# broadinstitute/permutect

Hardware: AMD Instinct MI355X
Metric: read-sets/sec (train fwd+bwd) (higher is better)
Workload: dtype f32 (fp32 accumulate; fwd: 2 x f16 pieces per operand = 23 bits; bwd: 2 x bf16 pieces = 16 bits)

## Files before the change

### permutect_amd/csrc/pmt_cnn3.hip

```cpp
#define PMT_OWN_WAVE_SHAPE
#define PMT_WAVES 8
#define PMT_RT 1
#include "pmt_device.hpp"

#ifndef C3_FWD_V
#define C3_FWD_V 4
#define C3_FWD_NW 8
#endif
#define C3_BWD_V 8
#define C3_BWD_NW 4
#define C3_MAXK 7
#define C3_NACC(K1, K2, L2) ((K1) * 2 + (K2) * 4 + (L2) * 2)
#define C3_NBIAS 80

struct C3Cfg {
    int S, K1, L1, P1, K2, L2, C1, C2, F, O;
    int st1, st2;
    int n1t, n2t, nPt;
    int act1, act2;
    int w1, b1, w2, b2, wl, bl;
    int per_wave;
    int stash_per;
};

DEV void c3_wave_sync() {
    asm volatile("s_waitcnt lgkmcnt(0)" ::: "memory");
    __builtin_amdgcn_wave_barrier();
}
DEV int c3_row(int m) { return 4 * (m & 3) + (m >> 2); }
DEV float c3_act(int kind, float x) { return kind == PMT_CNN_LEAKY_RELU ? fmaxf(x, 0.01f * x) : selu1(x); }
DEV float c3_act_grad(int kind, float y) { return kind == PMT_CNN_LEAKY_RELU ? (y > 0.f ? 1.f : 0.01f) : selu_grad_from_out(y); }
DEV f4 c3_act4(int kind, f4 v) { return f4{c3_act(kind, v[0]), c3_act(kind, v[1]), c3_act(kind, v[2]), c3_act(kind, v[3])}; }
DEV f4 c3_act_grad4(int kind, f4 y) { return f4{c3_act_grad(kind, y[0]), c3_act_grad(kind, y[1]), c3_act_grad(kind, y[2]), c3_act_grad(kind, y[3])}; }
DEV f4 c3_mfma4(f4 a, f4 b, f4 c) {
#pragma unroll
    for (int j = 0; j < 4; ++j) c = mfma16(a[j], b[j], c);
    return c;
}
DEV f4 c3_zero() { return f4{0.f, 0.f, 0.f, 0.f}; }
template <int CTRL>
DEV f4 c3_dpp4(f4 v) { return f4{dpp_mov<CTRL>(v[0]), dpp_mov<CTRL>(v[1]), dpp_mov<CTRL>(v[2]), dpp_mov<CTRL>(v[3])}; }

struct C3Weights {
    const float *w1f, *w2f, *wlf;
    const float *w2tf, *wltf;
    const float *b1p, *b2p, *blp;
};
DEV int c3_weight_floats(const C3Cfg& c, bool backward) {
    const int fwd = c.K1 * 2 * 256 + c.K2 * 4 * 256 + c.L2 * 2 * 256 + 80;
    const int bwd = c.K2 * 4 * 256 + c.L2 * 2 * 256;
    return backward ? bwd : fwd;
}
DEV C3Weights c3_build_weights(const C3Cfg& c, const float* __restrict__ theta, float* __restrict__ lds, bool backward) {
    C3Weights W{};
    const int tid = threadIdx.x, nthr = blockDim.x;
    float* cur = lds;
    if (!backward) {
        float* w1f = cur; cur += c.K1 * 2 * 256;
        for (int i = tid; i < c.K1 * 2 * 256; i += nthr) {
            const int j = i & 3, lane = (i >> 2) & 63, mt = (i >> 8) & 1, tap = i >> 9;
            const int co = 16 * mt + c3_row(lane & 15), ci = 4 * j + (lane >> 4);
            w1f[i] = (co < c.C1 && ci < 10) ? theta[c.w1 + (co * 10 + ci) * c.K1 + tap] : 0.f;
        }
        float* w2f = cur; cur += c.K2 * 4 * 256;
        for (int i = tid; i < c.K2 * 4 * 256; i += nthr) {
            const int j = i & 3, lane = (i >> 2) & 63, kt = (i >> 8) & 1, mt = (i >> 9) & 1, tap = i >> 10;
            const int co = 16 * mt + c3_row(lane & 15), ci = 16 * kt + 4 * j + (lane >> 4);
            w2f[i] = (co < c.C2 && ci < c.C1) ? theta[c.w2 + (co * c.C1 + ci) * c.K2 + tap] : 0.f;
        }
        float* wlf = cur; cur += c.L2 * 2 * 256;
        for (int i = tid; i < c.L2 * 2 * 256; i += nthr) {
            const int j = i & 3, lane = (i >> 2) & 63, t = (i >> 8) & 1, p = i >> 9;
            const int o = c3_row(lane & 15), ch = 16 * t + 4 * j + (lane >> 4);
            wlf[i] = (o < c.O && ch < c.C2) ? theta[c.wl + o * c.F + ch * c.L2 + p] : 0.f;
        }
        float* bp = cur; cur += 80;
        for (int i = tid; i < 80; i += nthr) {
            const int e = i & 15, f = 16 * ((i >> 4) & 1) + c3_row(e);
            float v = 0.f;
            if (i < 32) v = f < c.C1 ? theta[c.b1 + f] : 0.f;
            else if (i < 64) v = f < c.C2 ? theta[c.b2 + f] : 0.f;
            else v = c3_row(e) < c.O ? theta[c.bl + c3_row(e)] : 0.f;
            bp[i] = v;
        }
        W.w1f = w1f; W.w2f = w2f; W.wlf = wlf; W.b1p = bp; W.b2p = bp + 32; W.blp = bp + 64;
    } else {
        float* w2tf = cur; cur += c.K2 * 4 * 256;
        for (int i = tid; i < c.K2 * 4 * 256; i += nthr) {
            const int j = i & 3, lane = (i >> 2) & 63, kt = (i >> 8) & 1, mt = (i >> 9) & 1, tap = i >> 10;
            const int ci = 16 * mt + c3_row(lane & 15), co = 16 * kt + 4 * j + (lane >> 4);
            w2tf[i] = (co < c.C2 && ci < c.C1) ? theta[c.w2 + (co * c.C1 + ci) * c.K2 + tap] : 0.f;
        }
        float* wltf = cur; cur += c.L2 * 2 * 256;
        for (int i = tid; i < c.L2 * 2 * 256; i += nthr) {
            const int j = i & 3, lane = (i >> 2) & 63, t = (i >> 8) & 1, p = i >> 9;
            const int ch = 16 * t + c3_row(lane & 15), o = 4 * j + (lane >> 4);
            wltf[i] = (o < c.O && ch < c.C2) ? theta[c.wl + o * c.F + ch * c.L2 + p] : 0.f;
        }
        W.w2tf = w2tf; W.wltf = wltf;
    }
    __syncthreads();
    return W;
}

#define C3_COPY_F4 20
#define C3_HAP_LOADS 8
struct C3Wave {
    float* rec;
    int rec_floats, a2_off, arg_off;
    float* x;
    float* dout;
    unsigned char* hap;
    int P1, st2;
    DEV float* a1(int v, int q) const { return rec + v * rec_floats + q * 32; }
    DEV float* a2(int v, int p) const { return rec + v * rec_floats + a2_off + p * 32; }
    DEV unsigned* argb(int v, int q) const { return reinterpret_cast<unsigned*>(rec + v * rec_floats + arg_off) + q; }
};
template <int V>
DEV C3Wave c3_wave_region(const C3Cfg& c, float* base) {
    C3Wave w;
    w.rec = base;
    w.rec_floats = c.stash_per;
    w.a2_off = c.P1 * 32;
    w.arg_off = c.P1 * 32 + c.st2 * 32;
    w.P1 = c.P1; w.st2 = c.st2;
    w.x = base + V * c.stash_per;
    w.dout = w.x + V * c.st2 * 32;
    w.hap = reinterpret_cast<unsigned char*>(w.dout + V * 16);
    return w;
}
template <int V>
DEV void c3_load_haplotypes(const C3Cfg& c, const C3Wave& w, const long long* __restrict__ hap, long long hap_stride, long long v0, int nv) {
    const int lane = threadIdx.x & 63, n2s = 2 * c.S;
    long long b[C3_HAP_LOADS];
#pragma unroll
    for (int k = 0; k < C3_HAP_LOADS; ++k) {
        const int i = lane + 64 * k, v = i / n2s, e = i - v * n2s;
        b[k] = 255;
        if (i < V * n2s && v < nv) b[k] = hap[(size_t)(v0 + v) * hap_stride + e];
    }
#pragma unroll
    for (int k = 0; k < C3_HAP_LOADS; ++k) {
        const int i = lane + 64 * k;
        if (i < V * n2s) w.hap[i] = (b[k] >= 0 && b[k] < 5) ? (unsigned char)b[k] : (unsigned char)255;
    }
}
DEV void c3_store_records(const C3Wave& w, float* __restrict__ dst, int nv) {
    const int lane = threadIdx.x & 63, have = nv * w.rec_floats / 4;
#pragma unroll
    for (int k = 0; k < C3_COPY_F4; ++k) {
        const int i = lane + 64 * k;
        if (i < have) reinterpret_cast<f4*>(dst)[i] = reinterpret_cast<const f4*>(w.rec)[i];
    }
}
DEV f4 c3_one_hot(int S, const C3Wave& w, int v, int pos, int g) {
    const int base = w.hap[v * 2 * S + (g & 1) * S + pos];
    const int b0 = g >> 1;
    return f4{base == b0 ? 1.f : 0.f, base == b0 + 2 ? 1.f : 0.f, (g < 2 && base == b0 + 4) ? 1.f : 0.f, 0.f};
}

#ifndef C3_TRACE
#define C3_TRACE 0
#endif
#define C3_EV()                                                                                                      \
    do {                                                                                                             \
        if (C3_TRACE && tracing) { const unsigned long long t_ = __builtin_readcyclecounter(); if (lane == 0 && tr_n < 120) tr[tr_n] = t_; ++tr_n; } \
    } while (0)
template <int V, int NW, int K1, int K2, int L2, int S1>
__global__ __launch_bounds__(64 * NW, 1) void pmt_cnn3_forward_kernel(
    C3Cfg c, const float* __restrict__ theta, const long long* __restrict__ hap, long long hap_stride, int n, float* __restrict__ out,
    long long out_stride, float* __restrict__ stash) {
    extern __shared__ __attribute__((aligned(16))) float lds[];
    const unsigned long long t_begin = C3_TRACE ? __builtin_readcyclecounter() : 0ull;
    const C3Weights W = c3_build_weights(c, theta, lds, false);
    const unsigned long long t_weights = C3_TRACE ? __builtin_readcyclecounter() : 0ull;
    const int lane = threadIdx.x & 63, g = lane >> 4, r = lane & 15, wave = uniform((int)(threadIdx.x >> 6));
    bool tracing = false;
    unsigned long long* tr = reinterpret_cast<unsigned long long*>(stash);
    int tr_n = 2;
    const C3Wave w = c3_wave_region<V>(c, lds + ((c3_weight_floats(c, false) + 3) & ~3) + wave * c.per_wave);
    const int nbatches = (n + V - 1) / V;
    constexpr int P1 = L2 + K2 - 1, ST2 = L2 <= 4 ? 4 : 8, N2T = (V * ST2 + 15) / 16;
    const int S = S1 ? S1 : c.S, st1 = S1 ? ((S1 - K1 + 2) & ~1) : c.st1, n1t = S1 ? (V * st1 + 15) / 16 : c.n1t;
    const float inv_st1 = 1.0f / (float)st1;
    const f4 b1v[2] = {*reinterpret_cast<const f4*>(W.b1p + 4 * g), *reinterpret_cast<const f4*>(W.b1p + 16 + 4 * g)};
    const f4 b2v[2] = {*reinterpret_cast<const f4*>(W.b2p + 4 * g), *reinterpret_cast<const f4*>(W.b2p + 16 + 4 * g)};
    const f4 blv = *reinterpret_cast<const f4*>(W.blp + 4 * g);
    for (int batch = blockIdx.x * NW + wave; batch < nbatches; batch += gridDim.x * NW) {
        const long long v0 = (long long)batch * V;
        const int nv = (int)min((long long)V, (long long)n - v0);
        C3_EV();
        c3_load_haplotypes<V>(c, w, hap, hap_stride, v0, nv);
        c3_wave_sync();
        C3_EV();
#pragma unroll
        for (int T = 0; T < n1t; ++T) {
            const int col = 16 * T + r;
            int v = S1 ? col / st1 : (int)((float)col * inv_st1 + 1e-3f);
            int p = col - v * st1;
            const bool in_range = v < V;
            v = min(v, V - 1);
            f4 acc[2] = {b1v[0], b1v[1]};
#pragma unroll
            for (int tap = 0; tap < K1; ++tap) {
                const f4 b = c3_one_hot(S, w, v, min(p + tap, S - 1), g);
#pragma unroll
                for (int mt = 0; mt < 2; ++mt) {
                    const f4 a = *reinterpret_cast<const f4*>(W.w1f + ((tap * 2 + mt) * 64 + lane) * 4);
#pragma unroll
                    for (int j = 0; j < 3; ++j) acc[mt] = mfma16(a[j], b[j], acc[mt]);
                }
            }
            const int q = p >> 1;
            const bool store = in_range && !(p & 1) && q < P1;
            unsigned bits = 0;
#pragma unroll
            for (int mt = 0; mt < 2; ++mt) {
                const f4 nxt = c3_dpp4<0x101>(acc[mt]);
                f4 m;
#pragma unroll
                for (int j = 0; j < 4; ++j) {
                    const bool second = nxt[j] > acc[mt][j];
                    m[j] = second ? nxt[j] : acc[mt][j];
                    bits |= second ? 1u << (4 * mt + j) : 0u;
                }
                if (store) *reinterpret_cast<f4*>(w.a1(v, q) + 16 * mt + 4 * g) = c3_act4(c.act1, m);
            }
            if (store) reinterpret_cast<unsigned char*>(w.argb(v, q))[g] = (unsigned char)bits;
        }
        c3_wave_sync();
        C3_EV();
#pragma unroll
        for (int T = 0; T < N2T; ++T) {
            const int col = 16 * T + r;
            int v = col / ST2;
            const int p = col - v * ST2;
            const bool valid = v < V && p < L2;
            v = min(v, V - 1);
            f4 acc[2] = {b2v[0], b2v[1]};
#pragma unroll
            for (int tap = 0; tap < K2; ++tap) {
                const float* src = w.a1(v, min(p + tap, P1 - 1)) + 4 * g;
#pragma unroll
                for (int kt = 0; kt < 2; ++kt) {
                    const f4 b = *reinterpret_cast<const f4*>(src + 16 * kt);
#pragma unroll
                    for (int mt = 0; mt < 2; ++mt)
                        acc[mt] = c3_mfma4(*reinterpret_cast<const f4*>(W.w2f + (((tap * 2 + mt) * 2 + kt) * 64 + lane) * 4), b, acc[mt]);
                }
            }
            if (v < V && p < ST2 && col < V * ST2) {
#pragma unroll
                for (int mt = 0; mt < 2; ++mt) *reinterpret_cast<f4*>(w.a2(v, p) + 16 * mt + 4 * g) = valid ? c3_act4(c.act2, acc[mt]) : c3_zero();
            }
        }
        c3_wave_sync();
        C3_EV();
        {
            const int v = min(r, V - 1);
            f4 acc = blv;
#pragma unroll
            for (int p = 0; p < L2; ++p)
#pragma unroll
                for (int t = 0; t < 2; ++t)
                    acc = c3_mfma4(*reinterpret_cast<const f4*>(W.wlf + ((p * 2 + t) * 64 + lane) * 4),
                                   *reinterpret_cast<const f4*>(w.a2(v, p) + 16 * t + 4 * g), acc);
            if (r < nv) {
#pragma unroll
                for (int j = 0; j < 4; ++j)
                    if (4 * j + g < c.O) out[(size_t)(v0 + r) * out_stride + 4 * j + g] = acc[j];
            }
        }
        C3_EV();
        if (stash) {
            c3_wave_sync();
            c3_store_records(w, stash + (size_t)v0 * c.stash_per, nv);
        }
        c3_wave_sync();
        if (C3_TRACE && stash != nullptr && blockIdx.x == 0 && wave == 0) {
            asm volatile("s_waitcnt vmcnt(0)" ::: "memory");
            if (!tracing && lane == 0) { tr[0] = t_begin; tr[1] = t_weights; }
            tracing = true;
            C3_EV();
            if (lane == 0) tr[127] = (unsigned long long)tr_n;
        }
    }
}

#define C3B_OH_PAD 16
DEV int c3_chan_of_elem(int e) { return 16 * (e >> 4) + 4 * (e & 3) + ((e & 15) >> 2); }
typedef unsigned c3_u4 __attribute__((ext_vector_type(4)));
typedef unsigned c3_u2 __attribute__((ext_vector_type(2)));
typedef h8 c3p8;
#define C3_NP 2
#define C3_ONE ((unsigned short)0x3C00)
DEV f4 c3p_mfma(c3p8 a, c3p8 b, f4 c) { return mfma_f16(a, b, c); }
DEV void c3p_split(float a, float b, unsigned (&pc)[3]) {
    float k = 4096.f;
    asm volatile("" : "+v"(k));
    split_pair_f16(a, b, pc[0], pc[1], k);
    pc[2] = 0u;
}
DEV void c3p_mma(const c3p8 (&a)[C3_NP], const c3p8 (&b)[C3_NP], f4& acc, f4& lo) {
    lo = c3p_mfma(a[1], b[0], lo);
    lo = c3p_mfma(a[0], b[1], lo);
    acc = c3p_mfma(a[0], b[0], acc);
}
DEV f4 c3p_join(f4 acc, f4 lo) { return lo * (1.0f / 4096.f) + acc; }
#define C3_COL_BYTES (64 * C3_NP)
template <typename F>
DEV void c3b_build_frag(c3p8* __restrict__ dst, int ln, F value) {
    unsigned pc[4][3];
#pragma unroll
    for (int q = 0; q < 4; ++q) c3p_split(value(2 * q), value(2 * q + 1), pc[q]);
#pragma unroll
    for (int k = 0; k < C3_NP; ++k) dst[64 * k + ln] = __builtin_bit_cast(c3p8, c3_u4{pc[0][k], pc[1][k], pc[2][k], pc[3][k]});
}
DEV void c3b_store_pieces(unsigned char* dst, f4 v) {
    unsigned p0[3], p1[3];
    c3p_split(v[0], v[1], p0);
    c3p_split(v[2], v[3], p1);
#pragma unroll
    for (int k = 0; k < C3_NP; ++k) *reinterpret_cast<c3_u2*>(dst + 64 * k) = c3_u2{p0[k], p1[k]};
}
__host__ __device__ inline size_t c3b_wave_bytes(int V, int S, int P1, int ST2) {
    return (size_t)((V * (S * 10 + C3B_OH_PAD) * 2 + 15) & ~15) + (size_t)V * P1 * C3_COL_BYTES + (size_t)V * ST2 * C3_COL_BYTES;
}

template <int V, int NW, int K1, int K2, int L2, int S1, int A1, int A2, bool TRAIN>
__global__ __launch_bounds__(64 * NW, 1) void pmt_cnn3_forward_bf_kernel(
    C3Cfg c, const float* __restrict__ theta, const long long* __restrict__ hap, long long hap_stride, int n, float* __restrict__ out,
    long long out_stride, float* __restrict__ stash) {
    static_assert(K1 * 10 <= 32, "conv1's taps x channels are one k block");
    extern __shared__ __attribute__((aligned(16))) float lds[];
    constexpr int P1 = L2 + K2 - 1, ST2 = L2 <= 4 ? 4 : 8, N2T = (V * ST2 + 15) / 16;
    const int tid = threadIdx.x, lane = tid & 63, g = lane >> 4, r = lane & 15, wave = uniform((int)(tid >> 6));
    const int S = S1 ? S1 : c.S, st1 = S1 ? ((S1 - K1 + 2) & ~1) : c.st1, n1t = S1 ? (V * st1 + 15) / 16 : c.n1t;
    const float inv_st1 = 1.0f / (float)st1;
    const int OHS = S * 10 + C3B_OH_PAD;
    unsigned char* base = reinterpret_cast<unsigned char*>(lds);
    fp16_saturate_on();
    c3p8* wlb = reinterpret_cast<c3p8*>(base);
    float* bp = reinterpret_cast<float*>(base + L2 * C3_NP * 1024);
    unsigned char* dyn = base + L2 * C3_NP * 1024 + 320;
    c3p8* w1s = reinterpret_cast<c3p8*>(dyn);
    c3p8* w2s = w1s + 2 * 64 * C3_NP;
    for (int e = tid; e < 2 * 64; e += 64 * NW) {
        const int ln = e & 63, mt = e >> 6, co = 16 * mt + c3_row(ln & 15), kg = ln >> 4;
        c3b_build_frag(w1s + mt * 64 * C3_NP, ln, [&](int i) {
            const int k = 8 * kg + i, tap = k / 10, ci = k - 10 * tap;
            return (k < 10 * K1 && co < c.C1) ? theta[c.w1 + (co * 10 + ci) * K1 + tap] : 0.f;
        });
    }
    for (int e = tid; e < K2 * 2 * 64; e += 64 * NW) {
        const int ln = e & 63, tm = e >> 6, tap = tm >> 1, mt = tm & 1, co = 16 * mt + c3_row(ln & 15), kg = ln >> 4;
        c3b_build_frag(w2s + tm * 64 * C3_NP, ln, [&](int i) {
            const int ci = c3_chan_of_elem(8 * kg + i);
            return (co < c.C2 && ci < c.C1) ? theta[c.w2 + (co * c.C1 + ci) * K2 + tap] : 0.f;
        });
    }
    for (int e = tid; e < L2 * 64; e += 64 * NW) {
        const int ln = e & 63, p = e >> 6, o = c3_row(ln & 15), kg = ln >> 4;
        c3b_build_frag(wlb + p * 64 * C3_NP, ln, [&](int i) {
            const int ch = c3_chan_of_elem(8 * kg + i);
            return (o < c.O && ch < c.C2) ? theta[c.wl + o * c.F + ch * L2 + p] : 0.f;
        });
    }
    for (int i = tid; i < 80; i += 64 * NW) {
        const int e = i & 15, f = 16 * ((i >> 4) & 1) + c3_row(e);
        float v = 0.f;
        if (i < 32) v = f < c.C1 ? theta[c.b1 + f] : 0.f;
        else if (i < 64) v = f < c.C2 ? theta[c.b2 + f] : 0.f;
        else v = c3_row(e) < c.O ? theta[c.bl + c3_row(e)] : 0.f;
        bp[i] = v;
    }
    __syncthreads();
    c3p8 w1r[2][C3_NP], w2r[K2][2][C3_NP];
#pragma unroll
    for (int mt = 0; mt < 2; ++mt)
#pragma unroll
        for (int pc = 0; pc < C3_NP; ++pc) w1r[mt][pc] = w1s[(mt * C3_NP + pc) * 64 + lane];
#pragma unroll
    for (int tap = 0; tap < K2; ++tap)
#pragma unroll
        for (int mt = 0; mt < 2; ++mt)
#pragma unroll
            for (int pc = 0; pc < C3_NP; ++pc) w2r[tap][mt][pc] = w2s[((tap * 2 + mt) * C3_NP + pc) * 64 + lane];
    const f4 b1v[2] = {*reinterpret_cast<const f4*>(bp + 4 * g), *reinterpret_cast<const f4*>(bp + 16 + 4 * g)};
    const f4 b2v[2] = {*reinterpret_cast<const f4*>(bp + 32 + 4 * g), *reinterpret_cast<const f4*>(bp + 48 + 4 * g)};
    const f4 blv = *reinterpret_cast<const f4*>(bp + 64 + 4 * g);
    __syncthreads();
    unsigned char* oh = dyn + (size_t)wave * c3b_wave_bytes(V, S, P1, ST2);
    unsigned char* a1b = oh + ((V * OHS * 2 + 15) & ~15);
    unsigned char* a2b = a1b + V * P1 * C3_COL_BYTES;
    for (int i = lane; i < (V * OHS) / 2; i += 64) reinterpret_cast<unsigned*>(oh)[i] = 0u;
    c3_wave_sync();
    const int nbatches = (n + V - 1) / V, n2s = 2 * S;
    const int rec_a2 = P1 * 32, rec_arg = P1 * 32 + ST2 * 32;
    long long bnext[C3_HAP_LOADS];
    auto request = [&](int batch) {
        const long long v0 = (long long)batch * V;
#pragma unroll
        for (int k = 0; k < C3_HAP_LOADS; ++k) {
            const int i = lane + 64 * k, v = i / n2s, e = i - v * n2s;
            bnext[k] = 255;
            if (batch < nbatches && i < V * n2s && v0 + v < n) bnext[k] = hap[(size_t)(v0 + v) * hap_stride + e];
        }
    };
    request(blockIdx.x * NW + wave);
    for (int batch = blockIdx.x * NW + wave; batch < nbatches; batch += gridDim.x * NW) {
        const long long v0 = (long long)batch * V;
        const int nv = (int)min((long long)V, (long long)n - v0);
        {
            long long b[C3_HAP_LOADS];
#pragma unroll
            for (int k = 0; k < C3_HAP_LOADS; ++k) b[k] = bnext[k];
            request(batch + gridDim.x * NW);
#pragma unroll
            for (int k = 0; k < C3_HAP_LOADS; ++k) {
                const int i = lane + 64 * k, v = i / n2s, e = i - v * n2s, hs = e >= S ? 1 : 0, pos = e - hs * S;
                if (i < V * n2s) {
                    unsigned short* dst = reinterpret_cast<unsigned short*>(oh) + v * OHS + pos * 10 + hs;
#pragma unroll
                    for (int bs = 0; bs < 5; ++bs) dst[2 * bs] = b[k] == bs ? C3_ONE : (unsigned short)0;
                }
            }
        }
        c3_wave_sync();
        float* rec0 = TRAIN ? stash + (size_t)v0 * c.stash_per : nullptr;
#pragma unroll
        for (int T = 0; T < n1t; ++T) {
            const int col = 16 * T + r;
            int v = S1 ? col / st1 : (int)((float)col * inv_st1 + 1e-3f);
            const int p = col - v * st1;
            const bool in_range = v < V;
            v = min(v, V - 1);
            const unsigned* src = reinterpret_cast<const unsigned*>(oh + 2 * (v * OHS + p * 10 + 8 * g));
            const c3p8 b = __builtin_bit_cast(c3p8, c3_u4{src[0], src[1], src[2], src[3]});
            f4 acc[2] = {b1v[0], b1v[1]};
#pragma unroll
            for (int mt = 0; mt < 2; ++mt) {
                const f4 lo = c3p_mfma(w1r[mt][1], b, c3_zero());
                acc[mt] = c3p_join(c3p_mfma(w1r[mt][0], b, acc[mt]), lo);
            }
            const int q = p >> 1;
            const bool store = in_range && !(p & 1) && q < P1;
            unsigned bits = 0;
#pragma unroll
            for (int mt = 0; mt < 2; ++mt) {
                const f4 nxt = c3_dpp4<0x101>(acc[mt]);
                f4 m;
#pragma unroll
                for (int j = 0; j < 4; ++j) {
                    if constexpr (TRAIN) {
                        const bool second = nxt[j] > acc[mt][j];
                        m[j] = second ? nxt[j] : acc[mt][j];
                        bits |= second ? 1u << (4 * mt + j) : 0u;
                    } else {
                        m[j] = fmaxf(acc[mt][j], nxt[j]);
                    }
                }
                m = c3_act4(A1 ? A1 : c.act1, m);
                if (store) {
                    c3b_store_pieces(a1b + (v * P1 + q) * C3_COL_BYTES + (16 * mt + 4 * g) * 2, m);
                    if (TRAIN && v < nv) *reinterpret_cast<f4*>(rec0 + (size_t)v * c.stash_per + q * 32 + 16 * mt + 4 * g) = m;
                }
            }
            if (TRAIN && store && v < nv) reinterpret_cast<unsigned char*>(rec0 + (size_t)v * c.stash_per + rec_arg + q)[g] = (unsigned char)bits;
        }
        c3_wave_sync();
#pragma unroll
        for (int T = 0; T < N2T; ++T) {
            const int col = 16 * T + r;
            int v = col / ST2;
            const int p = col - v * ST2;
            const bool valid = v < V && p < L2;
            const bool in_range = v < V;
            v = min(v, V - 1);
            f4 acc[2] = {b2v[0], b2v[1]}, lo2[2] = {c3_zero(), c3_zero()};
#pragma unroll
            for (int tap = 0; tap < K2; ++tap) {
                const unsigned char* src = a1b + (v * P1 + min(p + tap, P1 - 1)) * C3_COL_BYTES + 16 * g;
                c3p8 b[C3_NP];
#pragma unroll
                for (int k = 0; k < C3_NP; ++k) b[k] = *reinterpret_cast<const c3p8*>(src + 64 * k);
#pragma unroll
                for (int mt = 0; mt < 2; ++mt) c3p_mma(w2r[tap][mt], b, acc[mt], lo2[mt]);
            }
#pragma unroll
            for (int mt = 0; mt < 2; ++mt) {
                const f4 a = valid ? c3_act4(A2 ? A2 : c.act2, c3p_join(acc[mt], lo2[mt])) : c3_zero();
                if (valid) c3b_store_pieces(a2b + (v * ST2 + p) * C3_COL_BYTES + (16 * mt + 4 * g) * 2, a);
                if (TRAIN && in_range && v < nv) *reinterpret_cast<f4*>(rec0 + (size_t)v * c.stash_per + rec_a2 + p * 32 + 16 * mt + 4 * g) = a;
            }
        }
        c3_wave_sync();
        {
            const int v = min(r, V - 1);
            f4 acc = blv, lol = c3_zero();
#pragma unroll
            for (int p = 0; p < L2; ++p) {
                const unsigned char* src = a2b + (v * ST2 + p) * C3_COL_BYTES + 16 * g;
                c3p8 b[C3_NP], a[C3_NP];
#pragma unroll
                for (int k = 0; k < C3_NP; ++k) {
                    b[k] = *reinterpret_cast<const c3p8*>(src + 64 * k);
                    a[k] = wlb[(p * C3_NP + k) * 64 + lane];
                }
                c3p_mma(a, b, acc, lol);
            }
            acc = c3p_join(acc, lol);
            if (r < nv) {
#pragma unroll
                for (int j = 0; j < 4; ++j)
                    if (4 * j + g < c.O) out[(size_t)(v0 + r) * out_stride + 4 * j + g] = acc[j];
            }
        }
        c3_wave_sync();
    }
}

#define C3T_POS 260
__host__ __device__ constexpr int c3w_max(int a, int b) { return a > b ? a : b; }
__host__ __device__ constexpr int c3w_a1t_floats(int P1) { return P1 * C3T_POS; }
__host__ __device__ constexpr int c3w_a2_floats(int V, int ST2) { return c3w_max(V * ST2 * 32, ST2 * C3T_POS); }
__host__ __device__ constexpr int c3w_arg_floats(int V, int P1) { return (V * P1 + 3) & ~3; }
__host__ __device__ constexpr int c3w_x_floats(int V, int ST2) { return V * ST2 * 32; }
#define C3T_OH_POS(V) (16 * (V) + 8)
__host__ __device__ constexpr int c3w_oh_floats(int V, int S) { return S * C3T_OH_POS(V) / 2; }
__host__ __device__ constexpr int c3w_floats(int V, int S, int P1, int ST2) {
    return c3w_a1t_floats(P1) + c3w_a2_floats(V, ST2) + c3w_arg_floats(V, P1) + c3w_x_floats(V, ST2) + V * 16 + c3w_oh_floats(V, S);
}
DEV void c3w_read8(const float* p, f4& lo, f4& hi) {
    lo = *reinterpret_cast<const f4*>(p);
    hi = *reinterpret_cast<const f4*>(p + 128);
}
DEV void c3w_split8(f4 lo, f4 hi, bf8& h, bf8& m) {
    unsigned hh[4], mm[4], unused = 0u;
    split_pair<2>(lo[0], lo[1], hh[0], mm[0], unused);
    split_pair<2>(lo[2], lo[3], hh[1], mm[1], unused);
    split_pair<2>(hi[0], hi[1], hh[2], mm[2], unused);
    split_pair<2>(hi[2], hi[3], hh[3], mm[3], unused);
    h = __builtin_bit_cast(bf8, c3_u4{hh[0], hh[1], hh[2], hh[3]});
    m = __builtin_bit_cast(bf8, c3_u4{mm[0], mm[1], mm[2], mm[3]});
}

template <int V, int NW, int K1, int K2, int L2>
__global__ __launch_bounds__(64 * NW, 1) void pmt_cnn3_backward_kernel(
    C3Cfg c, const float* __restrict__ theta, const long long* __restrict__ hap, long long hap_stride, int n, const float* __restrict__ d_out,
    long long d_out_stride, const float* __restrict__ stash, float* __restrict__ gtheta, float* __restrict__ ws, int ws_stride) {
    static_assert(V == 8, "a lane's eight consecutive k of a 32-deep block are the 8 variants of one position");
    extern __shared__ __attribute__((aligned(16))) float lds[];
    const unsigned long long t_begin = C3_TRACE ? __builtin_readcyclecounter() : 0ull;
    const C3Weights W = c3_build_weights(c, theta, lds, true);
    const unsigned long long t_weights = C3_TRACE ? __builtin_readcyclecounter() : 0ull;
    const int lane = threadIdx.x & 63, g = lane >> 4, r = lane & 15, wave = uniform((int)(threadIdx.x >> 6));
    const bool tracing = C3_TRACE && blockIdx.x == 0 && wave == 0;
    unsigned long long* tr = reinterpret_cast<unsigned long long*>(const_cast<float*>(stash));
    int tr_n = 2;
    const int m = r, kk = g;
    const int nbatches = (n + V - 1) / V;
    constexpr int P1 = L2 + K2 - 1, ST2 = L2 <= 4 ? 4 : 8, N2T = (V * ST2) / 16, NPT = (V * P1 + 15) / 16;
    constexpr int REC_A2 = P1 * 32, REC_ARG = P1 * 32 + ST2 * 32;
    static_assert(ST2 * C3T_POS <= c3w_a2_floats(V, ST2) && V * ST2 * 32 <= c3w_a2_floats(V, ST2), "a2 and the dY2 image share one array");
    static_assert(C3T_POS % 4 == 0 && C3T_POS >= 256 && c3w_a1t_floats(P1) % 4 == 0 && c3w_a2_floats(V, ST2) % 4 == 0, "16-byte operand reads");
    static_assert(ST2 % 4 == 0, "a k block is 4 positions");
    const int S = c.S;
    float* const a1t = lds + ((c3_weight_floats(c, true) + 3) & ~3) + wave * c3w_floats(V, S, P1, ST2);
    float* const a2 = a1t + c3w_a1t_floats(P1);
    float* const dyt = a2;
    unsigned* const argw = reinterpret_cast<unsigned*>(a2 + c3w_a2_floats(V, ST2));
    float* const x = reinterpret_cast<float*>(argw) + c3w_arg_floats(V, P1);
    float* const dout = x + c3w_x_floats(V, ST2);
    unsigned short* const oh = reinterpret_cast<unsigned short*>(dout + V * 16);
    for (int i = lane; i < c3w_oh_floats(V, S); i += 64) reinterpret_cast<unsigned*>(oh)[i] = 0u;
    c3_wave_sync();
    f4 gw1[K1][2], gw2[K2][2][2], gwl[L2][2];
    f4 gb1[2] = {c3_zero(), c3_zero()}, gb2[2] = {c3_zero(), c3_zero()};
    float gbl = 0.f;
#pragma unroll
    for (int k = 0; k < K1; ++k) gw1[k][0] = gw1[k][1] = c3_zero();
#pragma unroll
    for (int k = 0; k < K2; ++k) gw2[k][0][0] = gw2[k][0][1] = gw2[k][1][0] = gw2[k][1][1] = c3_zero();
#pragma unroll
    for (int k = 0; k < L2; ++k) gwl[k][0] = gwl[k][1] = c3_zero();
    constexpr int NA1 = (V * P1 * 8 + 63) / 64, NA2 = (V * ST2 * 8 + 63) / 64, NARG = (V * P1 + 63) / 64;
    const int n2s = 2 * S;
    long long hb[C3_HAP_LOADS];
    f4 t1[NA1], t2[NA2];
    unsigned ta[NARG];
    float td[(V * 16) / 64];
    int nv_req = 0;
    auto request = [&](int batch) {
        const int nv = batch < nbatches ? (int)min((long long)V, (long long)n - (long long)batch * V) : 0;
        const long long v0 = nv > 0 ? (long long)batch * V : 0;
        const float* src = stash + (size_t)v0 * c.stash_per;
#pragma unroll
        for (int k = 0; k < NA2; ++k) {
            const int i = min(lane + 64 * k, V * ST2 * 8 - 1), v = i / (ST2 * 8), rem = i - v * (ST2 * 8);
            t2[k] = *reinterpret_cast<const f4*>(src + (size_t)(v < nv ? v : 0) * c.stash_per + REC_A2 + 4 * rem);
        }
#pragma unroll
        for (int k = 0; k < (V * 16) / 64; ++k) {
            const int i = lane + 64 * k, v = i >> 4, o = i & 15;
            td[k] = d_out[(size_t)(v0 + (v < nv ? v : 0)) * d_out_stride + min(o, c.O - 1)];
        }
#pragma unroll
        for (int k = 0; k < NA1; ++k) {
            const int i = min(lane + 64 * k, V * P1 * 8 - 1), v = i / (P1 * 8), rem = i - v * (P1 * 8);
            t1[k] = *reinterpret_cast<const f4*>(src + (size_t)(v < nv ? v : 0) * c.stash_per + 4 * rem);
        }
#pragma unroll
        for (int k = 0; k < C3_HAP_LOADS; ++k) {
            const int i = min(lane + 64 * k, V * n2s - 1), v = i / n2s, e = i - v * n2s;
            hb[k] = hap[(size_t)(v0 + (v < nv ? v : 0)) * hap_stride + e];
        }
#pragma unroll
        for (int k = 0; k < NARG; ++k) {
            const int i = min(lane + 64 * k, V * P1 - 1), v = i / P1, q = i - v * P1;
            ta[k] = reinterpret_cast<const unsigned*>(src + (size_t)(v < nv ? v : 0) * c.stash_per + REC_ARG)[q];
        }
        nv_req = nv;
    };
    auto store_a2_dout = [&]() {
#pragma unroll
            for (int k = 0; k < NA2; ++k) {
                const int i = lane + 64 * k;
                if (i < V * ST2 * 8) reinterpret_cast<f4*>(a2)[i] = i / (ST2 * 8) < nv_req ? t2[k] : c3_zero();
            }
#pragma unroll
            for (int k = 0; k < (V * 16) / 64; ++k) {
                const int i = lane + 64 * k;
                dout[i] = ((i >> 4) < nv_req && (i & 15) < c.O) ? td[k] : 0.f;
            }
    };
    auto store_a1_arg_onehot = [&]() {
#pragma unroll
            for (int k = 0; k < C3_HAP_LOADS; ++k) {
                const int i = lane + 64 * k, v = i / n2s, e = i - v * n2s, hs = e >= S ? 1 : 0, pos = e - hs * S;
                if (i < V * n2s) {
                    unsigned short* dst = oh + pos * C3T_OH_POS(V) + hs * V + v;
#pragma unroll
                    for (int bs = 0; bs < 5; ++bs) dst[2 * bs * V] = (hb[k] == bs && v < nv_req) ? (unsigned short)0x3F80 : (unsigned short)0;
                }
            }
#pragma unroll
            for (int k = 0; k < NA1; ++k) {
                const int i = lane + 64 * k, v = i / (P1 * 8), rem = i - v * (P1 * 8), q = rem >> 3, e0 = (rem & 7) * 4;
                if (i < V * P1 * 8) {
                    float* dst = a1t + q * C3T_POS + (v >> 2) * 128 + e0 * 4 + (v & 3);
#pragma unroll
                    for (int j = 0; j < 4; ++j) dst[4 * j] = v < nv_req ? t1[k][j] : 0.f;
                }
            }
#pragma unroll
            for (int k = 0; k < NARG; ++k) {
                const int i = lane + 64 * k, v = i / P1, q = i - v * P1;
                if (i < V * P1) argw[q * V + v] = v < nv_req ? ta[k] : 0u;
            }
    };
    request(blockIdx.x * NW + wave);
    store_a2_dout();
    store_a1_arg_onehot();
    c3_wave_sync();
    for (int batch = blockIdx.x * NW + wave; batch < nbatches; batch += gridDim.x * NW) {
        if (C3_TRACE && tracing && lane == 0 && tr_n == 2) { tr[0] = t_begin; tr[1] = t_weights; }
        C3_EV();
        {
            const int v = min(r, V - 1);
            f4 bo;
#pragma unroll
            for (int j = 0; j < 4; ++j) bo[j] = (r < V) ? dout[v * 16 + 4 * j + g] : 0.f;
#pragma unroll
            for (int p = 0; p < L2; ++p)
#pragma unroll
                for (int t = 0; t < 2; ++t) {
                    const f4 d = c3_mfma4(*reinterpret_cast<const f4*>(W.wltf + ((p * 2 + t) * 64 + lane) * 4), bo, c3_zero());
                    if (r < V) *reinterpret_cast<f4*>(x + (v * ST2 + p) * 32 + 16 * t + 4 * g) = d;
                }
        }
        c3_wave_sync();
        C3_EV();
        for (int T = 0; T < N2T; ++T) {
            const int col = 16 * T + r;
            int v = col / ST2;
            const int p = col - v * ST2;
            const bool valid = v < V && p < L2;
            v = min(v, V - 1);
#pragma unroll
            for (int t = 0; t < 2; ++t) {
                float* px = x + (v * ST2 + p) * 32 + 16 * t + 4 * g;
                const f4 y = *reinterpret_cast<const f4*>(a2 + (v * ST2 + p) * 32 + 16 * t + 4 * g);
                f4 d = *reinterpret_cast<const f4*>(px) * c3_act_grad4(c.act2, y);
                if (!valid) d = c3_zero();
                if (v < V && col < V * ST2) *reinterpret_cast<f4*>(px) = d;
                gb2[t] = gb2[t] + d;
            }
        }
        {
#pragma unroll
            for (int s = 0; s < V / 4; ++s) {
                const int v = 4 * s + kk;
                const float a = dout[v * 16 + m];
                gbl += a;
#pragma unroll
                for (int p = 0; p < L2; ++p)
#pragma unroll
                    for (int t = 0; t < 2; ++t) gwl[p][t] = mfma16(a, a2[(v * ST2 + p) * 32 + 16 * t + m], gwl[p][t]);
            }
        }
        c3_wave_sync();
#pragma unroll
        for (int T = 0; T < N2T; ++T) {
            const int col = 16 * T + r, v = col / ST2, p = col - v * ST2;
#pragma unroll
            for (int t = 0; t < 2; ++t) {
                const f4 d = *reinterpret_cast<const f4*>(x + col * 32 + 16 * t + 4 * g);
                float* dst = dyt + p * C3T_POS + (v >> 2) * 128 + (16 * t + 4 * g) * 4 + (v & 3);
#pragma unroll
                for (int j = 0; j < 4; ++j) dst[4 * j] = d[j];
            }
        }
        c3_wave_sync();
        C3_EV();
        {
            constexpr int NB = ST2 / 4;
            f4 ra[NB][2][2], rb[NB][K2][2][2];
#pragma unroll
            for (int b = 0; b < NB; ++b) {
                const int p = 4 * b + kk;
#pragma unroll
                for (int mt = 0; mt < 2; ++mt) c3w_read8(dyt + p * C3T_POS + (16 * mt + m) * 4, ra[b][mt][0], ra[b][mt][1]);
#pragma unroll
                for (int tap = 0; tap < K2; ++tap)
#pragma unroll
                    for (int kt = 0; kt < 2; ++kt)
                        c3w_read8(a1t + min(p + tap, P1 - 1) * C3T_POS + (16 * kt + m) * 4, rb[b][tap][kt][0], rb[b][tap][kt][1]);
            }
#pragma unroll
            for (int b = 0; b < NB; ++b) {
                bf8 ah[2], am[2];
#pragma unroll
                for (int mt = 0; mt < 2; ++mt) c3w_split8(ra[b][mt][0], ra[b][mt][1], ah[mt], am[mt]);
#pragma unroll
                for (int tap = 0; tap < K2; ++tap)
#pragma unroll
                    for (int kt = 0; kt < 2; ++kt) {
                        bf8 bh, bm;
                        c3w_split8(rb[b][tap][kt][0], rb[b][tap][kt][1], bh, bm);
#pragma unroll
                        for (int mt = 0; mt < 2; ++mt) gw2[tap][mt][kt] = mfma_bf16(am[mt], bh, gw2[tap][mt][kt]);
#pragma unroll
                        for (int mt = 0; mt < 2; ++mt) gw2[tap][mt][kt] = mfma_bf16(ah[mt], bm, gw2[tap][mt][kt]);
#pragma unroll
                        for (int mt = 0; mt < 2; ++mt) gw2[tap][mt][kt] = mfma_bf16(ah[mt], bh, gw2[tap][mt][kt]);
                    }
            }
        }
        c3_wave_sync();
        C3_EV();
        request(batch + gridDim.x * NW);
#pragma unroll
        for (int T = 0; T < NPT; ++T) {
            const int idx = 16 * T + r;
            int v = idx / P1;
            const int q = idx - v * P1;
            const bool valid = v < V;
            v = min(v, V - 1);
            f4 acc[2] = {c3_zero(), c3_zero()};
#pragma unroll
            for (int tap = 0; tap < K2; ++tap) {
                const int p = q - tap;
                const bool ok = valid && p >= 0 && p < L2;
                const float* src = x + (v * ST2 + (ok ? p : 0)) * 32 + 4 * g;
#pragma unroll
                for (int kt = 0; kt < 2; ++kt) {
                    f4 b = *reinterpret_cast<const f4*>(src + 16 * kt);
                    if (!ok) b = c3_zero();
#pragma unroll
                    for (int mt = 0; mt < 2; ++mt)
                        acc[mt] = c3_mfma4(*reinterpret_cast<const f4*>(W.w2tf + (((tap * 2 + mt) * 2 + kt) * 64 + lane) * 4), b, acc[mt]);
                }
            }
            if (valid) {
#pragma unroll
                for (int mt = 0; mt < 2; ++mt) {
                    float* pa = a1t + q * C3T_POS + (v >> 2) * 128 + (16 * mt + 4 * g) * 4 + (v & 3);
                    const f4 d = acc[mt] * c3_act_grad4(c.act1, f4{pa[0], pa[4], pa[8], pa[12]});
#pragma unroll
                    for (int j = 0; j < 4; ++j) pa[4 * j] = d[j];
                    gb1[mt] = gb1[mt] + d;
                }
            }
        }
        c3_wave_sync();
        store_a2_dout();
        C3_EV();
        {
            constexpr int NB = (P1 + 3) / 4;
            f4 ra[NB][2][2];
            c3_u4 wa[NB][2];
            bf8 bo[NB][K1 + 1];
#pragma unroll
            for (int b = 0; b < NB; ++b) {
                const int q = min(4 * b + kk, P1 - 1);
#pragma unroll
                for (int mt = 0; mt < 2; ++mt) c3w_read8(a1t + q * C3T_POS + (16 * mt + m) * 4, ra[b][mt][0], ra[b][mt][1]);
                wa[b][0] = *reinterpret_cast<const c3_u4*>(argw + q * V);
                wa[b][1] = *reinterpret_cast<const c3_u4*>(argw + q * V + 4);
#pragma unroll
                for (int off = 0; off <= K1; ++off) bo[b][off] = *reinterpret_cast<const bf8*>(oh + min(2 * q + off, S - 1) * C3T_OH_POS(V) + m * V);
            }
#pragma unroll
            for (int b = 0; b < NB; ++b) {
                const bool valid = 4 * b + kk < P1;
#pragma unroll
                for (int mt = 0; mt < 2; ++mt) {
                    const int bit = 8 * (m >> 2) + 4 * mt + (m & 3);
                    f4 a0[2], a1[2];
#pragma unroll
                    for (int h = 0; h < 2; ++h)
#pragma unroll
                        for (int i = 0; i < 4; ++i) {
                            const float d = valid ? ra[b][mt][h][i] : 0.f;
                            const bool second = (wa[b][h][i] >> bit) & 1u;
                            a0[h][i] = second ? 0.f : d;
                            a1[h][i] = second ? d : 0.f;
                        }
                    bf8 a0h, a0m, a1h, a1m;
                    c3w_split8(a0[0], a0[1], a0h, a0m);
                    c3w_split8(a1[0], a1[1], a1h, a1m);
#pragma unroll
                    for (int tap = 0; tap < K1; ++tap) gw1[tap][mt] = mfma_bf16(a0m, bo[b][tap], gw1[tap][mt]);
#pragma unroll
                    for (int tap = 0; tap < K1; ++tap) gw1[tap][mt] = mfma_bf16(a0h, bo[b][tap], gw1[tap][mt]);
#pragma unroll
                    for (int tap = 0; tap < K1; ++tap) gw1[tap][mt] = mfma_bf16(a1m, bo[b][tap + 1], gw1[tap][mt]);
#pragma unroll
                    for (int tap = 0; tap < K1; ++tap) gw1[tap][mt] = mfma_bf16(a1h, bo[b][tap + 1], gw1[tap][mt]);
                }
            }
        }
        c3_wave_sync();
        store_a1_arg_onehot();
        c3_wave_sync();
        C3_EV();
    }
    if (ws != nullptr) {
        constexpr int NACC = C3_NACC(K1, K2, L2);
        __syncthreads();
        f4* red = reinterpret_cast<f4*>(lds);
        float* redb = lds + NW * NACC * 256;
        f4* mine = red + wave * NACC * 64 + lane;
#pragma unroll
        for (int tap = 0; tap < K1; ++tap)
#pragma unroll
            for (int mt = 0; mt < 2; ++mt) mine[(tap * 2 + mt) * 64] = gw1[tap][mt];
#pragma unroll
        for (int tap = 0; tap < K2; ++tap)
#pragma unroll
            for (int mt = 0; mt < 2; ++mt)
#pragma unroll
                for (int kt = 0; kt < 2; ++kt) mine[(K1 * 2 + (tap * 2 + mt) * 2 + kt) * 64] = gw2[tap][mt][kt];
#pragma unroll
        for (int p = 0; p < L2; ++p)
#pragma unroll
            for (int t = 0; t < 2; ++t) mine[(K1 * 2 + K2 * 4 + p * 2 + t) * 64] = gwl[p][t];
#pragma unroll
        for (int t = 0; t < 2; ++t)
#pragma unroll
            for (int j = 0; j < 4; ++j) {
                float s1 = gb1[t][j], s2 = gb2[t][j];
                s1 += dpp_mov<0xB1>(s1); s1 += dpp_mov<0x4E>(s1); s1 += dpp_mov<0x124>(s1); s1 += dpp_mov<0x128>(s1);
                s2 += dpp_mov<0xB1>(s2); s2 += dpp_mov<0x4E>(s2); s2 += dpp_mov<0x124>(s2); s2 += dpp_mov<0x128>(s2);
                if (r == 0) {
                    redb[wave * C3_NBIAS + 16 * t + 4 * j + g] = s1;
                    redb[wave * C3_NBIAS + 32 + 16 * t + 4 * j + g] = s2;
                }
            }
        {
            const float tot = group_sum(gbl);
            if (g == 0) redb[wave * C3_NBIAS + 64 + m] = tot;
        }
        __syncthreads();
        float* row = ws + (size_t)blockIdx.x * ws_stride;
        for (int a = wave; a < NACC; a += NW) {
            f4 sum = red[a * 64 + lane];
#pragma unroll
            for (int w2 = 1; w2 < NW; ++w2) sum = sum + red[(w2 * NACC + a) * 64 + lane];
            reinterpret_cast<f4*>(row)[a * 64 + lane] = sum;
        }
        if ((int)threadIdx.x < C3_NBIAS) {
            float sum = 0.f;
#pragma unroll
            for (int w2 = 0; w2 < NW; ++w2) sum += redb[w2 * C3_NBIAS + threadIdx.x];
            row[NACC * 256 + threadIdx.x] = sum;
        }
        if (C3_TRACE && tracing) {
            asm volatile("s_waitcnt vmcnt(0)" ::: "memory");
            C3_EV();
            if (lane == 0) tr[127] = (unsigned long long)tr_n;
        }
        return;
    }
#pragma unroll
    for (int tap = 0; tap < K1; ++tap)
#pragma unroll
        for (int mt = 0; mt < 2; ++mt)
#pragma unroll
            for (int j = 0; j < 4; ++j) {
                const int co = 16 * mt + c3_row(4 * g + j), ci = r;
                if (co < c.C1 && ci < 10) atomicAdd(&gtheta[c.w1 + (co * 10 + ci) * K1 + tap], gw1[tap][mt][j]);
            }
#pragma unroll
    for (int tap = 0; tap < K2; ++tap)
#pragma unroll
        for (int mt = 0; mt < 2; ++mt)
#pragma unroll
            for (int kt = 0; kt < 2; ++kt)
#pragma unroll
                for (int j = 0; j < 4; ++j) {
                    const int co = 16 * mt + c3_row(4 * g + j), ci = 16 * kt + c3_row(r);
                    if (co < c.C2 && ci < c.C1) atomicAdd(&gtheta[c.w2 + (co * c.C1 + ci) * K2 + tap], gw2[tap][mt][kt][j]);
                }
#pragma unroll
    for (int p = 0; p < L2; ++p)
#pragma unroll
        for (int t = 0; t < 2; ++t)
#pragma unroll
            for (int j = 0; j < 4; ++j) {
                const int o = 4 * g + j, ch = 16 * t + c3_row(r);
                if (o < c.O && ch < c.C2) atomicAdd(&gtheta[c.wl + o * c.F + ch * L2 + p], gwl[p][t][j]);
            }
#pragma unroll
    for (int t = 0; t < 2; ++t)
// ... 194 lines not shown
```

Baseline: 20.22 million.

## Use split-bf16 MFMA for backward data-gradient passes with prepacked weights

Backward weights (transposed conv2 and linear) are now prepacked in LDS as hi/mid bf16 pairs, and the dout->x and x->a1 gradient GEMMs use three bf16 MFMAs with K=8 instead of four fp32 16x16x1 MFMAs per element group. The activation-gradient result is kept in registers and written to a new packed bf16 hi/mid column layout (144-byte stride) so the conv2 transpose pass reads bf16 directly. This cuts fp32 MFMA issue count and LDS traffic but lowers gradient precision to roughly 16 bits and changes the x buffer layout and zero-padding handling.

```diff
diff --git a/permutect_amd/csrc/pmt_cnn3.hip b/permutect_amd/csrc/pmt_cnn3.hip
--- a/permutect_amd/csrc/pmt_cnn3.hip
+++ b/permutect_amd/csrc/pmt_cnn3.hip
@@ -28,6 +28,8 @@
     __builtin_amdgcn_wave_barrier();
 }
 DEV int c3_row(int m) { return 4 * (m & 3) + (m >> 2); }
+DEV int c3_chan_of_elem(int e) { return 16 * (e >> 4) + 4 * (e & 3) + ((e & 15) >> 2); }
+typedef unsigned c3_u4 __attribute__((ext_vector_type(4)));
 DEV float c3_act(int kind, float x) { return kind == PMT_CNN_LEAKY_RELU ? fmaxf(x, 0.01f * x) : selu1(x); }
 DEV float c3_act_grad(int kind, float y) { return kind == PMT_CNN_LEAKY_RELU ? (y > 0.f ? 1.f : 0.01f) : selu_grad_from_out(y); }
 DEV f4 c3_act4(int kind, f4 v) { return f4{c3_act(kind, v[0]), c3_act(kind, v[1]), c3_act(kind, v[2]), c3_act(kind, v[3])}; }
@@ -43,7 +45,7 @@
 
 struct C3Weights {
     const float *w1f, *w2f, *wlf;
-    const float *w2tf, *wltf;
+    const c3_u4 *w2tp, *wltp;
     const float *b1p, *b2p, *blp;
 };
 DEV int c3_weight_floats(const C3Cfg& c, bool backward) {
@@ -85,19 +87,41 @@
         }
         W.w1f = w1f; W.w2f = w2f; W.wlf = wlf; W.b1p = bp; W.b2p = bp + 32; W.blp = bp + 64;
     } else {
-        float* w2tf = cur; cur += c.K2 * 4 * 256;
-        for (int i = tid; i < c.K2 * 4 * 256; i += nthr) {
-            const int j = i & 3, lane = (i >> 2) & 63, kt = (i >> 8) & 1, mt = (i >> 9) & 1, tap = i >> 10;
-            const int ci = 16 * mt + c3_row(lane & 15), co = 16 * kt + 4 * j + (lane >> 4);
-            w2tf[i] = (co < c.C2 && ci < c.C1) ? theta[c.w2 + (co * c.C1 + ci) * c.K2 + tap] : 0.f;
-        }
-        float* wltf = cur; cur += c.L2 * 2 * 256;
-        for (int i = tid; i < c.L2 * 2 * 256; i += nthr) {
-            const int j = i & 3, lane = (i >> 2) & 63, t = (i >> 8) & 1, p = i >> 9;
-            const int ch = 16 * t + c3_row(lane & 15), o = 4 * j + (lane >> 4);
-            wltf[i] = (o < c.O && ch < c.C2) ? theta[c.wl + o * c.F + ch * c.L2 + p] : 0.f;
-        }
-        W.w2tf = w2tf; W.wltf = wltf;
+        c3_u4* w2tp = reinterpret_cast<c3_u4*>(cur); cur += c.K2 * 4 * 256;
+        for (int e = tid; e < c.K2 * 2 * 64; e += nthr) {
+            const int ln = e & 63, mt = (e >> 6) & 1, tap = e >> 7, ci = 16 * mt + c3_row(ln & 15), kg = ln >> 4;
+            unsigned h[4], md[4], unused = 0u;
+#pragma unroll
+            for (int q = 0; q < 4; ++q) {
+                float v[2];
+#pragma unroll
+                for (int s = 0; s < 2; ++s) {
+                    const int co = c3_chan_of_elem(8 * kg + 2 * q + s);
+                    v[s] = (co < c.C2 && ci < c.C1) ? theta[c.w2 + (co * c.C1 + ci) * c.K2 + tap] : 0.f;
+                }
+                split_pair<2>(v[0], v[1], h[q], md[q], unused);
+            }
+            w2tp[((tap * 2 + mt) * 2 + 0) * 64 + ln] = c3_u4{h[0], h[1], h[2], h[3]};
+            w2tp[((tap * 2 + mt) * 2 + 1) * 64 + ln] = c3_u4{md[0], md[1], md[2], md[3]};
+        }
+        c3_u4* wltp = reinterpret_cast<c3_u4*>(cur); cur += c.L2 * 2 * 256;
+        for (int e = tid; e < c.L2 * 2 * 32; e += nthr) {
+            const int ln = e & 31, t = (e >> 5) & 1, p = e >> 6, ch = 16 * t + c3_row(ln & 15), kg = ln >> 4;
+            unsigned h[4], md[4], unused = 0u;
+#pragma unroll
+            for (int q = 0; q < 4; ++q) {
+                float v[2];
+#pragma unroll
+                for (int s = 0; s < 2; ++s) {
+                    const int o = 8 * kg + 2 * q + s;
+                    v[s] = (o < c.O && ch < c.C2) ? theta[c.wl + o * c.F + ch * c.L2 + p] : 0.f;
+                }
+                split_pair<2>(v[0], v[1], h[q], md[q], unused);
+            }
+            wltp[((p * 2 + t) * 2 + 0) * 32 + ln] = c3_u4{h[0], h[1], h[2], h[3]};
+            wltp[((p * 2 + t) * 2 + 1) * 32 + ln] = c3_u4{md[0], md[1], md[2], md[3]};
+        }
+        W.w2tp = w2tp; W.wltp = wltp;
     }
     __syncthreads();
     return W;
@@ -288,8 +312,6 @@
 }
 
 #define C3B_OH_PAD 16
-DEV int c3_chan_of_elem(int e) { return 16 * (e >> 4) + 4 * (e & 3) + ((e & 15) >> 2); }
-typedef unsigned c3_u4 __attribute__((ext_vector_type(4)));
 typedef unsigned c3_u2 __attribute__((ext_vector_type(2)));
 typedef h8 c3p8;
 #define C3_NP 2
@@ -525,7 +547,9 @@
 __host__ __device__ constexpr int c3w_a1t_floats(int P1) { return P1 * C3T_POS; }
 __host__ __device__ constexpr int c3w_a2_floats(int V, int ST2) { return c3w_max(V * ST2 * 32, ST2 * C3T_POS); }
 __host__ __device__ constexpr int c3w_arg_floats(int V, int P1) { return (V * P1 + 3) & ~3; }
-__host__ __device__ constexpr int c3w_x_floats(int V, int ST2) { return V * ST2 * 32; }
+#define C3X_COL 144
+#define C3X_F (C3X_COL / 4)
+__host__ __device__ constexpr int c3w_x_floats(int V, int ST2) { return V * ST2 * C3X_F; }
 #define C3T_OH_POS(V) (16 * (V) + 8)
 __host__ __device__ constexpr int c3w_oh_floats(int V, int S) { return S * C3T_OH_POS(V) / 2; }
 __host__ __device__ constexpr int c3w_floats(int V, int S, int P1, int ST2) {
@@ -571,6 +595,7 @@
     float* const dyt = a2;
     unsigned* const argw = reinterpret_cast<unsigned*>(a2 + c3w_a2_floats(V, ST2));
     float* const x = reinterpret_cast<float*>(argw) + c3w_arg_floats(V, P1);
+    unsigned char* const xp = reinterpret_cast<unsigned char*>(x);
     float* const dout = x + c3w_x_floats(V, ST2);
     unsigned short* const oh = reinterpret_cast<unsigned short*>(dout + V * 16);
     for (int i = lane; i < c3w_oh_floats(V, S); i += 64) reinterpret_cast<unsigned*>(oh)[i] = 0u;
@@ -668,32 +693,34 @@
         C3_EV();
         {
             const int v = min(r, V - 1);
-            f4 bo;
-#pragma unroll
-            for (int j = 0; j < 4; ++j) bo[j] = (r < V) ? dout[v * 16 + 4 * j + g] : 0.f;
+            f4 bo0 = *reinterpret_cast<const f4*>(dout + v * 16 + 8 * (kk & 1)), bo1 = *reinterpret_cast<const f4*>(dout + v * 16 + 8 * (kk & 1) + 4);
+            if (r >= V || kk >= 2) bo0 = bo1 = c3_zero();
+            bf8 bh, bm;
+            c3w_split8(bo0, bo1, bh, bm);
 #pragma unroll
             for (int p = 0; p < L2; ++p)
 #pragma unroll
                 for (int t = 0; t < 2; ++t) {
-                    const f4 d = c3_mfma4(*reinterpret_cast<const f4*>(W.wltf + ((p * 2 + t) * 64 + lane) * 4), bo, c3_zero());
-                    if (r < V) *reinterpret_cast<f4*>(x + (v * ST2 + p) * 32 + 16 * t + 4 * g) = d;
+                    const c3_u4* a = W.wltp + (p * 2 + t) * 2 * 32 + (lane & 31);
+                    const bf8 ah = __builtin_bit_cast(bf8, a[0]), am = __builtin_bit_cast(bf8, a[32]);
+                    f4 d = mfma_bf16(am, bh, c3_zero());
+                    d = mfma_bf16(ah, bm, d);
+                    d = mfma_bf16(ah, bh, d);
+                    if (r < V) *reinterpret_cast<f4*>(x + (v * ST2 + p) * C3X_F + 16 * t + 4 * g) = d;
                 }
         }
         c3_wave_sync();
         C3_EV();
+        f4 dy[N2T][2];
+#pragma unroll
         for (int T = 0; T < N2T; ++T) {
-            const int col = 16 * T + r;
-            int v = col / ST2;
-            const int p = col - v * ST2;
-            const bool valid = v < V && p < L2;
-            v = min(v, V - 1);
+            const int col = 16 * T + r, p = col % ST2;
 #pragma unroll
             for (int t = 0; t < 2; ++t) {
-                float* px = x + (v * ST2 + p) * 32 + 16 * t + 4 * g;
-                const f4 y = *reinterpret_cast<const f4*>(a2 + (v * ST2 + p) * 32 + 16 * t + 4 * g);
-                f4 d = *reinterpret_cast<const f4*>(px) * c3_act_grad4(c.act2, y);
-                if (!valid) d = c3_zero();
-                if (v < V && col < V * ST2) *reinterpret_cast<f4*>(px) = d;
+                const f4 y = *reinterpret_cast<const f4*>(a2 + col * 32 + 16 * t + 4 * g);
+                f4 d = *reinterpret_cast<const f4*>(x + col * C3X_F + 16 * t + 4 * g) * c3_act_grad4(c.act2, y);
+                if (p >= L2) d = c3_zero();
+                dy[T][t] = d;
                 gb2[t] = gb2[t] + d;
             }
         }
@@ -715,10 +742,16 @@
             const int col = 16 * T + r, v = col / ST2, p = col - v * ST2;
 #pragma unroll
             for (int t = 0; t < 2; ++t) {
-                const f4 d = *reinterpret_cast<const f4*>(x + col * 32 + 16 * t + 4 * g);
+                const f4 d = dy[T][t];
                 float* dst = dyt + p * C3T_POS + (v >> 2) * 128 + (16 * t + 4 * g) * 4 + (v & 3);
 #pragma unroll
                 for (int j = 0; j < 4; ++j) dst[4 * j] = d[j];
+                unsigned h0, m0, h1, m1, unused = 0u;
+                split_pair<2>(d[0], d[1], h0, m0, unused);
+                split_pair<2>(d[2], d[3], h1, m1, unused);
+                unsigned char* px = xp + col * C3X_COL + (16 * t + 4 * g) * 2;
+                *reinterpret_cast<c3_u2*>(px) = c3_u2{h0, h1};
+                *reinterpret_cast<c3_u2*>(px + 64) = c3_u2{m0, m1};
             }
         }
         c3_wave_sync();
@@ -771,16 +804,25 @@
 #pragma unroll
             for (int tap = 0; tap < K2; ++tap) {
                 const int p = q - tap;
-                const bool ok = valid && p >= 0 && p < L2;
-                const float* src = x + (v * ST2 + (ok ? p : 0)) * 32 + 4 * g;
-#pragma unroll
-                for (int kt = 0; kt < 2; ++kt) {
-                    f4 b = *reinterpret_cast<const f4*>(src + 16 * kt);
-                    if (!ok) b = c3_zero();
-#pragma unroll
-                    for (int mt = 0; mt < 2; ++mt)
-                        acc[mt] = c3_mfma4(*reinterpret_cast<const f4*>(W.w2tf + (((tap * 2 + mt) * 2 + kt) * 64 + lane) * 4), b, acc[mt]);
-                }
+                const bool ok = p >= 0 && p < L2;
+                constexpr int ZERO_P = L2 < ST2 ? L2 : 0;
+                const unsigned char* src = xp + (v * ST2 + (ok ? p : ZERO_P)) * C3X_COL + 16 * kk;
+                c3_u4 bhw = *reinterpret_cast<const c3_u4*>(src), bmw = *reinterpret_cast<const c3_u4*>(src + 64);
+                if (L2 >= ST2 && !ok) bhw = bmw = c3_u4{0u, 0u, 0u, 0u};
+                const bf8 bh = __builtin_bit_cast(bf8, bhw), bm = __builtin_bit_cast(bf8, bmw);
+                bf8 ah[2], am[2];
+#pragma unroll
+                for (int mt = 0; mt < 2; ++mt) {
+                    const c3_u4* a = W.w2tp + (tap * 2 + mt) * 2 * 64 + lane;
+                    ah[mt] = __builtin_bit_cast(bf8, a[0]);
+                    am[mt] = __builtin_bit_cast(bf8, a[64]);
+                }
+#pragma unroll
+                for (int mt = 0; mt < 2; ++mt) acc[mt] = mfma_bf16(am[mt], bh, acc[mt]);
+#pragma unroll
+                for (int mt = 0; mt < 2; ++mt) acc[mt] = mfma_bf16(ah[mt], bm, acc[mt]);
+#pragma unroll
+                for (int mt = 0; mt < 2; ++mt) acc[mt] = mfma_bf16(ah[mt], bh, acc[mt]);
             }
             if (valid) {
 #pragma unroll
```

New measurement: 20.49 million (median of 6 runs). 1.01x the previous value.
